# mcahny/vps

Hardware: AMD Instinct MI355X
Metric: frames/sec FuseTrack 1024x2048 (higher is better)
Workload: dtype f32-grade: f16x3 split operands (fp16 pair with scaled residual, 22 significand bits) on MFMA, f32 accumulate

## Files before the change

vps_amd/csrc/corr_half.hip:

```cpp
#include "common.h"
#include "conv_common.h"

namespace {

__device__ __forceinline__ float bit_select(const unsigned m, const float a, const float b) {
    return __uint_as_float((m & __float_as_uint(a)) | (~m & __float_as_uint(b)));
}

template <int R, int NQ>
__global__ __launch_bounds__(256)
void correlation4h_kernel(const float* __restrict__ in1, int ld1, int coff1, const float* __restrict__ in2, int ld2, int coff2,
                          float* __restrict__ out, int out_ld, int out_coff, int N, int H, int W, int C, int act, float slope) {
    constexpr int D = 2 * R + 1, NCOL = D + 3, NSLOT = 4 * D, NIT = (D + 1) / 2;
    static_assert(NSLOT <= 64 && NSLOT > 32, "slots (displacement, pixel) of one row: folded from 64");
    const int lane = threadIdx.x & 63, hl = lane & 31, half = lane >> 5;
    const int wave = threadIdx.x >> 6;
    const int gpr = W >> 2;
    const int ngroups = N * H * gpr;
    const int c4n = C >> 2;
    const float invC = 1.0f / (float)C;
    const __amdgpu_buffer_rsrc_t r1 = make_rsrc(in1, (unsigned)((size_t)N * H * W * ld1 * sizeof(float)));
    const __amdgpu_buffer_rsrc_t r2 = make_rsrc(in2, (unsigned)((size_t)N * H * W * ld2 * sizeof(float)));
    unsigned choff[NQ];
    bool chok[NQ];
#pragma unroll
    for (int q = 0; q < NQ; ++q) { chok[q] = hl + 32 * q < c4n; choff[q] = 16u * (unsigned)(hl + 32 * q); }
    int mine = 0;
#pragma unroll
    for (int s = 0; s < 5; ++s) mine += (lane >> (4 - s) & 1) ? 32 >> s : 0;
    const int my_ti = mine >> 2, my_p = mine & 3;

    const int gstep = (int)gridDim.x * 4;
    int grp = (int)blockIdx.x * 4 + wave;
    int g = grp % gpr, y, n;
    { const int t = grp / gpr; y = t % H; n = t / H; }
    const int dq = gstep / gpr, dr = gstep - dq * gpr;
    for (; grp < ngroups; grp += gstep) {
        const int xb = 4 * g;
        const unsigned pix = (unsigned)((n * H + y) * W + xb);
        f32x4 a[4][NQ];
#pragma unroll
        for (int p = 0; p < 4; ++p)
#pragma unroll
            for (int q = 0; q < NQ; ++q)
                a[p][q] = buffer_load16<f32x4>(r1, chok[q] ? (pix + p) * (unsigned)ld1 * 4u + (unsigned)coff1 * 4u + choff[q] : 0xFFFFFFF0u, 0u);
#pragma unroll 1
        for (int it = 0; it < NIT; ++it) {
            const int tj = 2 * it + half - R;
            const int y2 = y + tj;
            const bool rowok = tj <= R && (unsigned)y2 < (unsigned)H;
            const unsigned row2 = (unsigned)((n * H + y2) * W) * (unsigned)ld2 * 4u + (unsigned)coff2 * 4u;
            float v[64];
#pragma unroll
            for (int i = NSLOT; i < 64; ++i) v[i] = 0.f;
#pragma unroll
            for (int cb = 0; cb < NCOL; cb += 6) {
                f32x4 b[6][NQ];
#pragma unroll
                for (int du = 0; du < 6; ++du) {
                    const int uu = cb + du;
                    if (uu >= NCOL) continue;
                    const int x2 = xb + uu - R;
                    const bool ok = rowok && (unsigned)x2 < (unsigned)W;
#pragma unroll
                    for (int q = 0; q < NQ; ++q)
                        b[du][q] = buffer_load16<f32x4>(r2, (ok && chok[q]) ? row2 + (unsigned)x2 * (unsigned)ld2 * 4u + choff[q] : 0xFFFFFFF0u, 0u);
                }
                __builtin_amdgcn_sched_barrier(0);
#pragma unroll
                for (int du = 0; du < 6; ++du) {
                    const int uu = cb + du;
                    if (uu >= NCOL) continue;
#pragma unroll
                    for (int p = 0; p < 4; ++p) {
                        const int ti = uu - p;
                        if (ti < 0 || ti >= D) continue;
                        float acc = a[p][0][0] * b[du][0][0];
                        acc = __builtin_fmaf(a[p][0][1], b[du][0][1], acc);
                        acc = __builtin_fmaf(a[p][0][2], b[du][0][2], acc);
                        acc = __builtin_fmaf(a[p][0][3], b[du][0][3], acc);
#pragma unroll
                        for (int q = 1; q < NQ; ++q)
#pragma unroll
                            for (int e = 0; e < 4; ++e) acc = __builtin_fmaf(a[p][q][e], b[du][q][e], acc);
                        v[ti * 4 + p] = acc;
                    }
                }
            }
#pragma unroll
            for (int s = 0; s < 5; ++s) {
                const int off = 16 >> s, hf = 32 >> s;
                const unsigned up = (lane & off) ? 0xFFFFFFFFu : 0u;
#pragma unroll
                for (int i = 0; i < hf; ++i) {
                    if (s == 0 && i + hf >= NSLOT) { v[i] += __shfl_xor(v[i], off, 64); continue; }
                    const float send = bit_select(up, v[i], v[i + hf]);
                    const float keep = bit_select(up, v[i + hf], v[i]);
                    v[i] = keep + __shfl_xor(send, off, 64);
                }
            }
            if (tj <= R && my_ti < D) {
                float* __restrict__ o = out + ((size_t)pix + my_p) * out_ld + out_coff + (tj + R) * D + my_ti;
                o[0] = vps_act(v[0] * invC, act, slope);
                o[out_ld] = vps_act(v[1] * invC, act, slope);
            }
        }
        g += dr; y += dq;
        if (g >= gpr) { g -= gpr; ++y; }
        while (y >= H) { y -= H; ++n; }
    }
}

}

__attribute__((visibility("hidden")))
bool vpsi_launch_corr4h(const float* in1, int ld1, int coff1, const float* in2, int ld2, int coff2, float* out, int out_ld, int out_coff,
                        int N, int H, int W, int C, int r, int stride2, int act, float slope, hipStream_t s) {
    const char* e = getenv("VPS_CORR_HALF");
    if (e && e[0] == '0') return false;
    if (stride2 != 1 || r != 4 || (W & 3) || C > 256 || (C & 3)) return false;
    if ((size_t)N * H * W * ld1 * 4 >= 0xFFFFFFF0ull || (size_t)N * H * W * ld2 * 4 >= 0xFFFFFFF0ull || (long)N * H * (W / 4) >= 0x7fffffffL) return false;
    long g4 = ((long)N * H * (W / 4) + 3) / 4; if (g4 > 2048) g4 = 2048;
    if (C <= 128) hipLaunchKernelGGL((correlation4h_kernel<4, 1>), dim3((unsigned)g4), dim3(256), 0, s, in1, ld1, coff1, in2, ld2, coff2, out, out_ld, out_coff, N, H, W, C, act, slope);
    else hipLaunchKernelGGL((correlation4h_kernel<4, 2>), dim3((unsigned)g4), dim3(256), 0, s, in1, ld1, coff1, in2, ld2, coff2, out, out_ld, out_coff, N, H, W, C, act, slope);
    return true;
}
```

Before: 57.17.

## Replace shuffle-based slot reduction with permlane16 swap and DPP row folds

```diff
diff --git a/vps_amd/csrc/corr_half.hip b/vps_amd/csrc/corr_half.hip
--- a/vps_amd/csrc/corr_half.hip
+++ b/vps_amd/csrc/corr_half.hip
@@ -7,28 +7,50 @@
     return __uint_as_float((m & __float_as_uint(a)) | (~m & __float_as_uint(b)));
 }
 
+template <int CTRL>
+__device__ __forceinline__ float row_dpp(const float x) {
+    return __int_as_float(__builtin_amdgcn_update_dpp(0, __float_as_int(x), CTRL, 0xF, 0xF, true));
+}
+constexpr int DPP_ROW_MIRROR = 0x140;
+constexpr int DPP_ROW_HALF_MIRROR = 0x141;
+constexpr int DPP_QUAD_MIRROR = 0x1B;
+constexpr int DPP_QUAD_XOR1 = 0xB1;
+
+template <int CTRL>
+__device__ __forceinline__ void fold_row(float* v, const int hf, const int real, const unsigned up) {
+#pragma unroll
+    for (int i = 0; i < hf; ++i) {
+        const float lo = v[i] + row_dpp<CTRL>(v[i]);
+        if (i >= real) { v[i] = lo; continue; }
+        const float hi = v[i + hf] + row_dpp<CTRL>(v[i + hf]);
+        v[i] = bit_select(up, hi, lo);
+    }
+}
+
 template <int R, int NQ>
 __global__ __launch_bounds__(256)
 void correlation4h_kernel(const float* __restrict__ in1, int ld1, int coff1, const float* __restrict__ in2, int ld2, int coff2,
                           float* __restrict__ out, int out_ld, int out_coff, int N, int H, int W, int C, int act, float slope) {
     constexpr int D = 2 * R + 1, NCOL = D + 3, NSLOT = 4 * D, NIT = (D + 1) / 2;
-    static_assert(NSLOT <= 64 && NSLOT > 32, "slots (displacement, pixel) of one row: folded from 64");
-    const int lane = threadIdx.x & 63, hl = lane & 31, half = lane >> 5;
-    const int wave = threadIdx.x >> 6;
+    static_assert(NSLOT == 36, "slots (displacement, pixel) of one row: 36 -> 18 -> 16 -> 8 -> 4 -> 2 per lane");
+    const int lane = threadIdx.x & 63, half = lane >> 5;
+    const int hl = (lane & 16) | ((lane ^ (lane >> 1)) & 7) | (lane & 8);
+    const int wave = __builtin_amdgcn_readfirstlane(threadIdx.x >> 6);
     const int gpr = W >> 2;
     const int ngroups = N * H * gpr;
     const int c4n = C >> 2;
     const float invC = 1.0f / (float)C;
     const __amdgpu_buffer_rsrc_t r1 = make_rsrc(in1, (unsigned)((size_t)N * H * W * ld1 * sizeof(float)));
     const __amdgpu_buffer_rsrc_t r2 = make_rsrc(in2, (unsigned)((size_t)N * H * W * ld2 * sizeof(float)));
+    constexpr unsigned OUTSIDE = 0xFFFFFFF0u;
     unsigned choff[NQ];
-    bool chok[NQ];
 #pragma unroll
-    for (int q = 0; q < NQ; ++q) { chok[q] = hl + 32 * q < c4n; choff[q] = 16u * (unsigned)(hl + 32 * q); }
-    int mine = 0;
-#pragma unroll
-    for (int s = 0; s < 5; ++s) mine += (lane >> (4 - s) & 1) ? 32 >> s : 0;
+    for (int q = 0; q < NQ; ++q) choff[q] = hl + 32 * q < c4n ? 16u * (unsigned)(hl + 32 * q) : OUTSIDE;
+    const int mine = 18 * (hl >> 4) + 2 * (hl & 15);
+    const bool mine_ok = (hl & 15) <= 8;
     const int my_ti = mine >> 2, my_p = mine & 3;
+    const unsigned up8 = (hl & 8) ? 0xFFFFFFFFu : 0u, up4 = (hl & 4) ? 0xFFFFFFFFu : 0u;
+    const unsigned up2 = (hl & 2) ? 0xFFFFFFFFu : 0u, up1 = (hl & 1) ? 0xFFFFFFFFu : 0u;
 
     const int gstep = (int)gridDim.x * 4;
     int grp = (int)blockIdx.x * 4 + wave;
@@ -43,16 +65,23 @@
         for (int p = 0; p < 4; ++p)
 #pragma unroll
             for (int q = 0; q < NQ; ++q)
-                a[p][q] = buffer_load16<f32x4>(r1, chok[q] ? (pix + p) * (unsigned)ld1 * 4u + (unsigned)coff1 * 4u + choff[q] : 0xFFFFFFF0u, 0u);
+                a[p][q] = buffer_load16<f32x4>(r1, __builtin_elementwise_add_sat((pix + p) * (unsigned)ld1 * 4u + (unsigned)coff1 * 4u, choff[q]), 0u);
+        unsigned coloff[NCOL];
+#pragma unroll
+        for (int uu = 0; uu < NCOL; ++uu) {
+            const int x2 = xb + uu - R;
+            coloff[uu] = (unsigned)x2 < (unsigned)W ? (unsigned)x2 * (unsigned)ld2 * 4u : OUTSIDE;
+        }
 #pragma unroll 1
         for (int it = 0; it < NIT; ++it) {
             const int tj = 2 * it + half - R;
             const int y2 = y + tj;
             const bool rowok = tj <= R && (unsigned)y2 < (unsigned)H;
-            const unsigned row2 = (unsigned)((n * H + y2) * W) * (unsigned)ld2 * 4u + (unsigned)coff2 * 4u;
-            float v[64];
+            unsigned rowbase[NQ];
 #pragma unroll
-            for (int i = NSLOT; i < 64; ++i) v[i] = 0.f;
+            for (int q = 0; q < NQ; ++q)
+                rowbase[q] = rowok ? __builtin_elementwise_add_sat((unsigned)((n * H + y2) * W) * (unsigned)ld2 * 4u + (unsigned)coff2 * 4u, choff[q]) : OUTSIDE;
+            float v[NSLOT];
 #pragma unroll
             for (int cb = 0; cb < NCOL; cb += 6) {
                 f32x4 b[6][NQ];
@@ -60,11 +89,9 @@
                 for (int du = 0; du < 6; ++du) {
                     const int uu = cb + du;
                     if (uu >= NCOL) continue;
-                    const int x2 = xb + uu - R;
-                    const bool ok = rowok && (unsigned)x2 < (unsigned)W;
 #pragma unroll
                     for (int q = 0; q < NQ; ++q)
-                        b[du][q] = buffer_load16<f32x4>(r2, (ok && chok[q]) ? row2 + (unsigned)x2 * (unsigned)ld2 * 4u + choff[q] : 0xFFFFFFF0u, 0u);
+                        b[du][q] = buffer_load16<f32x4>(r2, __builtin_elementwise_add_sat(rowbase[q], coloff[uu]), 0u);
                 }
                 __builtin_amdgcn_sched_barrier(0);
 #pragma unroll
@@ -88,18 +115,15 @@
                 }
             }
 #pragma unroll
-            for (int s = 0; s < 5; ++s) {
-                const int off = 16 >> s, hf = 32 >> s;
-                const unsigned up = (lane & off) ? 0xFFFFFFFFu : 0u;
-#pragma unroll
-                for (int i = 0; i < hf; ++i) {
-                    if (s == 0 && i + hf >= NSLOT) { v[i] += __shfl_xor(v[i], off, 64); continue; }
-                    const float send = bit_select(up, v[i], v[i + hf]);
-                    const float keep = bit_select(up, v[i + hf], v[i]);
-                    v[i] = keep + __shfl_xor(send, off, 64);
-                }
+            for (int i = 0; i < NSLOT / 2; ++i) {
+                const auto sw = __builtin_amdgcn_permlane16_swap(__float_as_uint(v[i]), __float_as_uint(v[i + NSLOT / 2]), false, false);
+                v[i] = __uint_as_float(sw[0]) + __uint_as_float(sw[1]);
             }
-            if (tj <= R && my_ti < D) {
+            fold_row<DPP_ROW_MIRROR>(v, 16, NSLOT / 2 - 16, up8);
+            fold_row<DPP_ROW_HALF_MIRROR>(v, 8, 8, up4);
+            fold_row<DPP_QUAD_MIRROR>(v, 4, 4, up2);
+            fold_row<DPP_QUAD_XOR1>(v, 2, 2, up1);
+            if (tj <= R && mine_ok) {
                 float* __restrict__ o = out + ((size_t)pix + my_p) * out_ld + out_coff + (tj + R) * D + my_ti;
                 o[0] = vps_act(v[0] * invC, act, slope);
                 o[out_ld] = vps_act(v[1] * invC, act, slope);
```

After: 57.29, median of 6. Within noise of the previous version (+0.2%).
